# AlexandreDubray/consistent-viterbi

Measured on AMD Instinct MI355X. Metric: trellis cells/s (N*T*batch), N=256 T=512 batch=65536, higher is better.
Workload: dtype f64

## Files before the change

### consistent-viterbi_amd/csrc/cviterbi.cpp

```cpp
#include <hip/hip_runtime.h>

#include <algorithm>
#include <atomic>
#include <charconv>
#include <chrono>
#include <cmath>
#include <cstdarg>
#include <cstdio>
#include <cstdlib>
#include <cstring>
#include <memory>
#include <functional>
#include <limits>
#include <mutex>
#include <numeric>
#include <string>
#include <thread>
#include <type_traits>
#include <vector>

#include "../../include/cviterbi.h"
#include "batchplan.hpp"
#include "csp.hpp"
#include "hostscan.hpp"
// ... 3978 lines not shown
  return CV_OK;
}

CV_API int32_t cv_last_t64_stats(const cv_hmm* h, int64_t* out, int32_t n) {
  if (!h || n < 0 || (n > 0 && !out)) {
    set_err(CV_EINVAL, "bad argument");
    return -1;
  }
  int64_t v[8];
  t64_stats_sum(h, v);
  for (int32_t q = 0; q < n && q < 8; ++q) out[q] = v[q];
  return 8;
}

CV_API int32_t cv_last_fixed_first_stats(const cv_hmm* h, int64_t* out, int32_t n) {
  if (!h || n < 0 || (n > 0 && !out)) {
    set_err(CV_EINVAL, "bad argument");
    return -1;
  }
  for (int32_t q = 0; q < n && q < 4; ++q) out[q] = h->fx_last[q];
  return 4;
}

CV_API int32_t cv_last_first_pass_kind(const cv_hmm* h) {
  if (!h) {
    set_err(CV_EINVAL, "null handle");
    return -1;
  }
  return h->fx_last_kind;
}

CV_API cv_status cv_f32ru_trace(cv_hmm* h, int64_t nseq, int64_t T, const int32_t* obs, float* rows, float* mu,
                                float* r, float* e_last, int32_t* path) {
  if (!h || !obs || !rows || !mu || !r || !e_last || !path) return set_err(CV_EINVAL, "null argument");
  if (nseq < 2 || T < 1 || nseq * T > (1 << 22)) return set_err(CV_EINVAL, "bad batch shape");
  CV_LOCK(h);
  cv_status st = set_device(h);
  if (st != CV_OK) return st;
  for (int64_t e = 0; e < nseq * T; ++e)
    if (obs[e] < 0 || obs[e] >= h->V) return set_err(CV_EINVAL, "observation out of range");
  if ((st = ensure_ru_tables(h)) != CV_OK) return st;
  if (h->ru_state != 1) return set_err(CV_EINVAL, "the model is outside the round-up pass's range");
  const int np = cvk::trellis_padded_states(h->N);
  const size_t ne = (size_t)(nseq * T);
  std::vector<int64_t> off((size_t)nseq + 1);
  for (int64_t s = 0; s <= nseq; ++s) off[(size_t)s] = s * T;
  DevBuf d_off, d_obs, d_rows, d_mu, d_r, d_e, d_path, d_cert;
  if ((st = upload(d_off, off.data(), off.size() * 8)) != CV_OK) return st;
  if ((st = upload(d_obs, obs, ne * 4)) != CV_OK) return st;
  if ((st = d_rows.ensure(ne * np * 4)) != CV_OK) return st;
  if ((st = d_mu.ensure(ne * 4)) != CV_OK) return st;
  if ((st = d_r.ensure(ne * 4)) != CV_OK) return st;
  if ((st = d_e.ensure((size_t)nseq * 4)) != CV_OK) return st;
  if ((st = d_path.ensure(ne * 4)) != CV_OK) return st;
  if ((st = d_cert.ensure((size_t)nseq)) != CV_OK) return st;
  hipStream_t stream = h->stream;
  HIP_TRY(hipMemsetAsync(d_cert.p, 0, (size_t)nseq, stream));
  HIP_TRY(hipMemsetAsync(d_mu.p, 0, ne * 4, stream));
  HIP_TRY(hipMemsetAsync(d_r.p, 0, ne * 4, stream));
  HIP_TRY(hipMemsetAsync(d_rows.p, 0, ne * np * 4, stream));
  HIP_TRY(hipMemsetAsync(d_path.p, 0, ne * 4, stream));
  HIP_TRY(hipMemsetAsync(d_e.p, 0, (size_t)nseq * 4, stream));
  cvk::RuFwdArgs fa{};
  fa.a_img = h->ru_aimg.as<float>();
  fa.pi = h->ru_pi.as<float>();
  fa.et = h->ru_et.as<float>();
  fa.offsets = d_off.as<int64_t>();
  fa.obs = d_obs.as<int32_t>();
  fa.rows = d_rows.as<float>();
  fa.mu = d_mu.as<float>();
  fa.cert = d_cert.as<uint8_t>();
  fa.nobs = (int)h->V;
  hipError_t err = cvk::launch_ru_fwd2(np, fa, nseq / 2, stream);
  cvk::RuBtArgs ba{};
  ba.rows = fa.rows;
  ba.at = h->ru_at.as<float>();
  ba.offsets = fa.offsets;
  ba.seq_end = nseq - (nseq & 1);
  ba.path = d_path.as<int32_t>();
// ... 1631 lines not shown
```

### consistent-viterbi_amd/csrc/kernels/trellis.h

```cpp
#pragma once
#include <hip/hip_runtime.h>
#include <stdint.h>

namespace cvk {

enum { CVK_SEQ_OK = 0, CVK_SEQ_INFEASIBLE = 1, CVK_SEQ_EMPTY = 2, CVK_SEQ_BADOBS = 3 };
enum { CVK_ASSOC_VITERBI = 0, CVK_ASSOC_CP = 1, CVK_ASSOC_DP = 2, CVK_ASSOC_DECODE = 3 };

struct TrellisFwdArgs {
  const float* a_img;
  const float* pi;
  const float* et;
  const int64_t* offsets;
  const int32_t* obs;
  const int32_t* order;
  int64_t seq_begin;
  float* delta;
  int64_t delta_elem_base;
  uint8_t* status;
  int nobs;
  const int32_t* forced;
  const int64_t* ranges;
  int reverse;
  float* last_row;
// ... 96 lines not shown
  int nobs;
};
struct RuBtArgs {
  const float* rows;
  int64_t row_elem_base;
  const float* at;
  const int64_t* offsets;
  const int32_t* order;
  int64_t seq_begin, seq_end;
  int32_t* path;
  float* r;
  float* e_last;
  uint8_t* cert;
};
struct RuScoreArgs {
  const int32_t* path;
  const int32_t* obs;
  const int64_t* offsets;
  int64_t seq_begin, seq_end;
  int nstates;
  const double* pi64;
  const double* a64;
  const double* et64;
  const double* ca;
  const double* cb;
  const float* mu;
  const float* r;
  const float* e_last;
  double ks;
  uint8_t* cert;
  double* score;
  uint8_t* status;
};
hipError_t launch_ru_fwd2(int np, const RuFwdArgs& fa, int64_t npairs, hipStream_t stream);
hipError_t launch_ru_bt(int np, const RuBtArgs& ba, hipStream_t stream, int lds_reserve = 0);
hipError_t launch_ru_score(const RuScoreArgs& r, hipStream_t stream, int lds_reserve = 0);

template <typename REAL>
struct GenericFwdArgs {
  const int32_t* forced;
  const REAL* a;
  const REAL* pi;
  const REAL* et;
  const int64_t* offsets;
  const int32_t* obs;
  const int32_t* order;
  int64_t seq_begin;
  int nstates, nobs, assoc;
  uint16_t* psi;
  int64_t psi_elem_base;
  REAL* last_row;
  uint8_t* status;
  REAL* rows;
  const REAL* cp_init;
  REAL* cp_last;
  REAL* grows;
  int64_t wide_steps;
  int prio;
};

template <typename REAL>
struct GenericBtArgs {
  const uint16_t* psi;
  int64_t psi_elem_base;
  const REAL* last_row;
  const int64_t* offsets;
// ... 91 lines not shown
```

### consistent-viterbi_amd/csrc/kernels/trellis.hip

```cpp
#include <hip/hip_runtime.h>
#include <stdint.h>
#include <stdlib.h>

#include <algorithm>

#include "trellis.h"
#include "../tuning.h"

namespace cvk {

__device__ __forceinline__ float ninf_f() { return -__builtin_inff(); }

__device__ __forceinline__ float octet_max(float x) {
  asm volatile(
      "s_nop 1\n\t"
      "v_max_f32_dpp %0, %0, %0 quad_perm:[1,0,3,2] row_mask:0xf bank_mask:0xf\n\t"
      "s_nop 1\n\t"
      "v_max_f32_dpp %0, %0, %0 quad_perm:[2,3,0,1] row_mask:0xf bank_mask:0xf\n\t"
      "s_nop 1\n\t"
      "v_max_f32_dpp %0, %0, %0 row_half_mirror row_mask:0xf bank_mask:0xf"
      : "+v"(x));
  return x;
}

__device__ __forceinline__ float swap_max(float x, bool sixteen) {
  float a = x, b = x;
  if (sixteen)
    asm volatile("s_nop 1\n\tv_permlane16_swap_b32 %0, %1" : "+v"(a), "+v"(b));
  else
    asm volatile("s_nop 1\n\tv_permlane32_swap_b32 %0, %1" : "+v"(a), "+v"(b));
  return fmaxf(a, b);
}

__device__ __forceinline__ float wave_max(float x) {
  x = octet_max(x);
  asm volatile(
      "s_nop 1\n\t"
// ... 1015 lines not shown
}

hipError_t launch_fix_bt(int np, const FixBtArgs& ba, hipStream_t stream, int lds_reserve) {
  const int64_t n = ba.seq_end - ba.seq_begin;
  if (n <= 0) return hipSuccess;
  if (np != 256) return hipErrorInvalidValue;
  if (lds_reserve > 0)
    (void)hipFuncSetAttribute(reinterpret_cast<const void*>(&backtrack_fix_i32<256>),
                              hipFuncAttributeMaxDynamicSharedMemorySize, 160 * 1024);
  hipLaunchKernelGGL((backtrack_fix_i32<256>), dim3((unsigned)((n + 3) / 4)), dim3(256), (size_t)lds_reserve, stream,
                     ba);
  return hipGetLastError();
}

hipError_t launch_fix_score(const FixScoreArgs& r, hipStream_t stream, int lds_reserve) {
  const int64_t n = r.seq_end - r.seq_begin;
  if (n <= 0) return hipSuccess;
  if (lds_reserve > 0)
    (void)hipFuncSetAttribute(reinterpret_cast<const void*>(&fix_score_f64), hipFuncAttributeMaxDynamicSharedMemorySize,
                              160 * 1024);
  hipLaunchKernelGGL(fix_score_f64, dim3((unsigned)((n + 63) / 64)), dim3(64), (size_t)lds_reserve, stream, r);
  return hipGetLastError();
}

__device__ __forceinline__ void round_f32_up() {
  __builtin_amdgcn_s_setreg(1 | (1 << 11), 1);
  asm volatile("" ::: "memory");
}
__device__ __forceinline__ float dpp_max_half_mirror(float x) {
  asm volatile("s_nop 1\n\tv_max_f32_dpp %0, %0, %0 row_half_mirror row_mask:0xf bank_mask:0xf" : "+v"(x));
  return x;
}

template <int NP>
__global__ __launch_bounds__(NP * 4) void trellis_fwd2_f32ru(RuFwdArgs args) {
  using G = TrellisGeom<NP>;
  constexpr int R = G::R;
  constexpr int S = G::S;
  static_assert(R % 8 == 0, "pair kernel needs NP % 64 == 0");
  __shared__ __attribute__((aligned(16))) float lds[2][2][G::LDS_FLOATS];
  __shared__ float mu[2][3];
  round_f32_up();

  const int lane = threadIdx.x & 63;
  const int w = threadIdx.x >> 6;
  const int rg = lane & 7;
  const int cp = lane >> 3;
  const int j0 = 16 * w + 2 * cp;
  const bool hi = rg >= 4;
  const unsigned jw = (unsigned)(j0 + (hi ? 1 : 0));

  const int64_t slot = args.seq_begin + 2 * (int64_t)blockIdx.x;
  const int64_t seqX = args.order ? (int64_t)args.order[slot] : slot;
  const int64_t seqY = args.order ? (int64_t)args.order[slot + 1] : slot + 1;
  const int64_t eX = args.offsets[seqX], eY = args.offsets[seqY];
  const int T = (int)(args.offsets[seqX + 1] - eX);
  if (T <= 0) return;
  typedef const __attribute__((address_space(4))) int32_t* cobs_t;
  const cobs_t obsX = (cobs_t)(args.obs + eX);
  const cobs_t obsY = (cobs_t)(args.obs + eY);
  float* const dX = args.rows + (eX - args.row_elem_base) * NP;
  float* const dY = args.rows + (eY - args.row_elem_base) * NP;
  float* const muX = args.mu + eX;
  float* const muY = args.mu + eY;
  const unsigned V = (unsigned)args.nobs;

  if (threadIdx.x < 6) (&mu[0][0])[threadIdx.x] = ninf_f();
  __builtin_amdgcn_s_setprio(3);
// ... 26 lines not shown
  auto clampT = [&](int t) { return t < T ? t : T - 1; };
  typedef __attribute__((address_space(3))) float* lds_float_t;
  auto post_max = [&](float v, float* dst) {
    const float m = dpp_max_half_mirror(v);
    if (rg == 0) asm volatile("ds_max_f32 %0, %1" : : "v"((unsigned)(size_t)(lds_float_t)dst), "v"(m) : "memory");
  };
  lds_barrier();

  float eXr;
  {
    const float ex = et_row(obs_x(0)), ey = et_row(obs_y(0));
    const float p = args.pi[jw];
    eXr = et_row(obs_x(clampT(1)));
    const float dx = p + ex, dy = p + ey;
    lds[0][0][lds_w] = dx;
    lds[1][0][lds_w] = dy;
    dX[jw] = dx;
    dY[jw] = dy;
    post_max(dx, &mu[0][0]);
    post_max(dy, &mu[1][0]);
  }
  float eYr;
  unsigned oY = obs_y(clampT(1));
  unsigned oX = obs_x(clampT(2));
  lds_barrier();
  constexpr int KB = R / 8;
  auto ld8 = [&](const float* src, float4 (&dst)[2]) {
    dst[0] = *reinterpret_cast<const float4*>(src);
    dst[1] = *reinterpret_cast<const float4*>(src + 4);
  };
  float4 P[2], Q[2];
  ld8(&lds[0][0][rg * S], P);

  auto half = [&](const float* dsrc, const float* nsrc, float* ldst, float* drow, float* mus, float* mrow, int t,
                  const float& e_use, float& e_load, unsigned& o_load, bool first, int t_obs) {
    e_load = et_row(o_load);
    const float mu_use = fmaxf(mus[(t + 2) % 3], -__FLT_MAX__);
    if (threadIdx.x == 0) mus[(t + 1) % 3] = ninf_f();
    if (KB > 1) ld8(dsrc + 8, Q);
    float m0a = ninf_f(), m0b = ninf_f(), m1a = ninf_f(), m1b = ninf_f();
    auto rows4 = [&](const float4& dd, int k, bool init) {
      const float s00 = dd.x + a_reg[2 * k + 0], s01 = dd.x + a_reg[2 * k + 1];
      const float s10 = dd.y + a_reg[2 * k + 2], s11 = dd.y + a_reg[2 * k + 3];
      const float s20 = dd.z + a_reg[2 * k + 4], s21 = dd.z + a_reg[2 * k + 5];
      const float s30 = dd.w + a_reg[2 * k + 6], s31 = dd.w + a_reg[2 * k + 7];
      if (init) {
        m0a = fmaxf(s00, s10);
        m1a = fmaxf(s01, s11);
        m0b = fmaxf(s20, s30);
        m1b = fmaxf(s21, s31);
      } else {
        m0a = fmaxf(fmaxf(m0a, s00), s10);
        m1a = fmaxf(fmaxf(m1a, s01), s11);
        m0b = fmaxf(fmaxf(m0b, s20), s30);
        m1b = fmaxf(fmaxf(m1b, s21), s31);
      }
    };
#pragma unroll
    for (int k = 0; k < KB; ++k) {
      float4(&B)[2] = (k & 1) ? Q : P;
      rows4(B[0], 8 * k, k == 0);
      rows4(B[1], 8 * k + 4, false);
      __builtin_amdgcn_sched_barrier(0);
      if (k + 2 < KB)
        ld8(dsrc + 8 * (k + 2), B);
      else if (!(k & 1) && (k + 2 == KB || k + 1 == KB) && !first)
        ld8(nsrc, P);
      __builtin_amdgcn_sched_barrier(0);
    }
    const float m0 = fmaxf(m0a, m0b);
    const float m1 = fmaxf(m1a, m1b);
    float m = dpp_max_mirror(hi ? m1 : m0, hi ? m0 : m1);
    m = dpp_max_xor1(m);
    m = dpp_max_xor2(m);
    const float dn = (m + e_use) - mu_use;
    __builtin_amdgcn_sched_barrier(0);
    o_load = first ? obs_y(t_obs) : obs_x(t_obs);
    ldst[lds_w] = dn;
    (drow + (size_t)t * NP)[jw] = dn;
    mrow[t] = mu_use;
    post_max(dn, &mus[t % 3]);
    if (first) {
      lds_barrier();
      ld8(nsrc, P);
    }
  };
  auto step = [&](int t) {
    const int cur = (t - 1) & 1, nxt = t & 1;
    half(&lds[0][cur][rg * S], &lds[1][cur][rg * S], &lds[0][nxt][0], dX, mu[0], muX, t, eXr, eYr, oY, true,
         clampT(t + 1));
    half(&lds[1][cur][rg * S], &lds[0][nxt][rg * S], &lds[1][nxt][0], dY, mu[1], muY, t, eYr, eXr, oX, false,
         clampT(t + 2));
  };
  for (int t = 1; t < T; ++t) step(t);
  if (bad && lane == 0 && w == 0) {
    if (bad & 1u) args.cert[seqX] = CVK_SEQ_BADOBS;
    if (bad & 2u) args.cert[seqY] = CVK_SEQ_BADOBS;
  }
}

template <int NP>
__global__ __launch_bounds__(256) void backtrack_f32ru(RuBtArgs args) {
  constexpr int VL = NP / 64;
  constexpr int PF = 8;
  static_assert(VL == 4, "float4 rows");
  round_f32_up();
  const int lane = threadIdx.x & 63;
  const int64_t slot = args.seq_begin + (int64_t)blockIdx.x * 4 + (threadIdx.x >> 6);
  if (slot >= args.seq_end) return;
  const int64_t seq = args.order ? (int64_t)args.order[slot] : slot;
  const int64_t e0 = args.offsets[seq];
  const int T = (int)(args.offsets[seq + 1] - e0);
  if (T <= 0 || args.cert[seq] != 0) return;
  int32_t* __restrict__ path = args.path + e0;
  float* __restrict__ rout = args.r + e0;
  const float* __restrict__ drow = args.rows + (e0 - args.row_elem_base) * NP + VL * lane;
  const float* __restrict__ at = args.at + VL * lane;
  auto load_row = [&](int r, float (&dst)[VL]) {
    if (r >= 0) {
      ld_vl<VL>(drow + (size_t)r * NP, dst);
    } else {
      dst[0] = dst[1] = dst[2] = dst[3] = ninf_f();
    }
  };
  auto top2 = [&](const float (&s)[VL], float& M2) -> int {
    const float M = wave_max(fmaxf(fmaxf(s[0], s[1]), fmaxf(s[2], s[3])));
    const int win = first_argmax_vl<VL>(s, M, lane) & (NP - 1);
// ... 50 lines not shown
  const int32_t* __restrict__ obs = r.obs + e0;
  const float* __restrict__ mu = r.mu + e0;
  const float* __restrict__ rr = r.r + e0;
  const int N = r.nstates;
  auto absfin = [](double x) { return __builtin_isinf(x) ? 0.0 : __builtin_fabs(x); };
  auto sigma = [&](int n, double s) { return r.ks * (((double)n + 2.0) * ((double)n + 2.0)) + 0x1p-49 * s; };
  int pp = path[0];
  double L = r.pi64[pp] + r.et64[(size_t)obs[0] * N + pp];
  double C = r.cb[obs[0]];
  bool ok = true;
  for (int t = 1; t < T; ++t) {
    const int p = path[t];
    const int o = obs[t];
    const double rt = (double)rr[t], cap = r.ca[p];
    const double lhs = L + r.a64[(size_t)pp * N + p];
    const double rhs = (rt + cap) + C;
    ok = ok && (lhs - rhs > sigma(t, absfin(rt) + __builtin_fabs(cap) + __builtin_fabs(C) + __builtin_fabs(lhs)));
    L = lhs + r.et64[(size_t)o * N + p];
    const double ct = r.cb[o], mt = (double)mu[t];
    const double s = __builtin_fabs(C) + __builtin_fabs(ct) + __builtin_fabs(mt);
    C = ((C + ct) + mt) + 0x1p-50 * s;
    pp = p;
  }
  const double E = (double)r.e_last[seq];
  ok = ok && (L - (E + C) > sigma(T, absfin(E) + __builtin_fabs(C) + __builtin_fabs(L)));
  if (ok) {
    r.score[seq] = L;
    r.status[seq] = CVK_SEQ_OK;
  } else {
    r.cert[seq] = 2;
  }
}

hipError_t launch_ru_fwd2(int np, const RuFwdArgs& fa, int64_t npairs, hipStream_t stream) {
  if (npairs <= 0) return hipSuccess;
  if (np != 256) return hipErrorInvalidValue;
  hipLaunchKernelGGL((trellis_fwd2_f32ru<256>), dim3((unsigned)npairs), dim3(1024), 0, stream, fa);
  return hipGetLastError();
}

hipError_t launch_ru_bt(int np, const RuBtArgs& ba, hipStream_t stream, int lds_reserve) {
  const int64_t n = ba.seq_end - ba.seq_begin;
  if (n <= 0) return hipSuccess;
  if (np != 256) return hipErrorInvalidValue;
  if (lds_reserve > 0)
    (void)hipFuncSetAttribute(reinterpret_cast<const void*>(&backtrack_f32ru<256>),
                              hipFuncAttributeMaxDynamicSharedMemorySize, 160 * 1024);
  hipLaunchKernelGGL((backtrack_f32ru<256>), dim3((unsigned)((n + 3) / 4)), dim3(256), (size_t)lds_reserve, stream, ba);
  return hipGetLastError();
}

hipError_t launch_ru_score(const RuScoreArgs& r, hipStream_t stream, int lds_reserve) {
  const int64_t n = r.seq_end - r.seq_begin;
  if (n <= 0) return hipSuccess;
  if (lds_reserve > 0)
    (void)hipFuncSetAttribute(reinterpret_cast<const void*>(&ru_score_f64), hipFuncAttributeMaxDynamicSharedMemorySize,
                              160 * 1024);
  hipLaunchKernelGGL(ru_score_f64, dim3((unsigned)((n + 63) / 64)), dim3(64), (size_t)lds_reserve, stream, r);
  return hipGetLastError();
}

template <int NPW, bool FRC>
__global__ __launch_bounds__(256) void trellis_wave_f32(TrellisFwdArgs args, BacktrackArgs bargs) {
  constexpr int C = NPW / 16;
  constexpr int R = NPW / 4;
  constexpr int LS = R + 4;
  static_assert(NPW % 16 == 0 && NPW >= 16 && NPW <= 64, "NPW in {16, 32, 48, 64}");
  __shared__ __attribute__((aligned(16))) float lds_all[4][2][4 * LS];
  __shared__ __attribute__((aligned(16))) float at_lds[NPW * NPW];
  for (int k = threadIdx.x; k < NPW * NPW; k += 256) at_lds[k] = bargs.at[k];
// ... 1410 lines not shown
```

### consistent-viterbi_amd/csrc/tuning.cpp

```cpp
#include "tuning.h"

#include <cctype>
#include <cstdlib>
#include <cstring>
#include <string>

namespace cvk {
namespace {

struct Key {
  const char* name;
  int Tuning::*field;
};

#define CVK_KEY(f) {#f, &Tuning::f}
const Key kKeys[] = {
    CVK_KEY(trace), CVK_KEY(host_threads), CVK_KEY(t64_nonpos), CVK_KEY(generic_rows),
    CVK_KEY(max_chunks), CVK_KEY(emis_overlap), CVK_KEY(host_sums), CVK_KEY(no_trace), CVK_KEY(no_resume),
    CVK_KEY(no_side), CVK_KEY(chain_par), CVK_KEY(chain_old), CVK_KEY(chain_par_force),
    CVK_KEY(chain_spec), CVK_KEY(chain_spec_kernel), CVK_KEY(chain_copy_overlap), CVK_KEY(chain_cert_fused),
    CVK_KEY(chain_parts), CVK_KEY(chain_tail), CVK_KEY(chain_tail_div), CVK_KEY(chain_spec_prio), CVK_KEY(chain_pin_obs), CVK_KEY(chain_pin_path), CVK_KEY(t64_s),
    CVK_KEY(t64_512), CVK_KEY(t64_1024), CVK_KEY(t64_wg), CVK_KEY(t64_wg_force),
    CVK_KEY(t64_rs), CVK_KEY(t64_w2), CVK_KEY(t64_wave), CVK_KEY(t64_bal),
    CVK_KEY(t64_cp_s), CVK_KEY(t64_cp_w), CVK_KEY(t64_cp_pf), CVK_KEY(t64_bt_pf),
    CVK_KEY(t64_lo_every), CVK_KEY(t64_fixed_first), CVK_KEY(t64_fixed_chunks), CVK_KEY(t64_few),
    CVK_KEY(t64_f32ru_first),
    CVK_KEY(generic_s), CVK_KEY(generic_split), CVK_KEY(generic_split_k), CVK_KEY(generic_wide),
    CVK_KEY(generic_wide_min), CVK_KEY(generic_prio), CVK_KEY(wide_s), CVK_KEY(ext_wide_min),
    CVK_KEY(chain_wide), CVK_KEY(chain_wide_min), CVK_KEY(f32_onebar), CVK_KEY(bw_global),
    CVK_KEY(bw_perseq), CVK_KEY(bw_gemm_path), CVK_KEY(bw_chunk_elems), CVK_KEY(bw_max_waves),
    CVK_KEY(xi_part_rows),
};
#undef CVK_KEY

const Key* find(const char* key) {
  if (!key) return nullptr;
  for (const Key& k : kKeys)
    if (std::strcmp(k.name, key) == 0) return &k;
  return nullptr;
}

const Tuning kDefaults{};
thread_local const Tuning* t_cur = nullptr;
thread_local Tuning t_copy;
thread_local int t_depth = 0;

}

const Tuning& tuning() { return t_cur ? *t_cur : kDefaults; }

void tuning_enter(const Tuning& t) {
  if (t_depth++ == 0) {
    t_copy = t;
    t_cur = &t_copy;
  }
}

void tuning_leave() {
  if (t_depth > 0 && --t_depth == 0) t_cur = nullptr;
// ... 46 lines not shown
```

### consistent-viterbi_amd/csrc/tuning.h

```cpp
#pragma once

#include <cstdint>

namespace cvk {

struct Tuning {
  int trace = 0;
  int host_threads = 0;
  int t64_nonpos = 1;
  int generic_rows = 1;
  int max_chunks = 8;
  int emis_overlap = 0;
  int host_sums = 0;
  int no_trace = 0;
  int no_resume = 0;
  int no_side = 0;
  int chain_par = 1;
  int chain_old = 0;
  int chain_par_force = 0;
  int chain_spec = 1;
  int chain_spec_kernel = 0;
  int chain_copy_overlap = 1;
  int chain_cert_fused = 1;
  int chain_parts = 1;
  int chain_tail = 2;
  int chain_tail_div = 2;
  int chain_spec_prio = 3;
  int chain_pin_obs = 0;
  int chain_pin_path = 0;
  int t64_s = 0;
  int t64_512 = -1;
  int t64_1024 = -1;
  int t64_wg = 1;
  int t64_wg_force = 0;
  int t64_rs = 1;
  int t64_w2 = 1;
  int t64_few = -1;
  int t64_wave = 1;
  int t64_bal = 8;
  int t64_cp_s = 0;
  int t64_cp_pf = 0;
  int t64_cp_w = 0;
  int t64_bt_pf = 0;
  int t64_lo_every = 8;
  int t64_fixed_first = 16777216;
  int t64_f32ru_first = 16777216;
  int t64_fixed_chunks = 8;
  int generic_s = 0;
  int generic_split = 0;
  int generic_split_k = 0;
  int generic_wide = 1;
  int generic_wide_min = 0;
  int generic_prio = 0;
  int wide_s = 0;
  int ext_wide_min = 0;
  int chain_wide = 1;
  int chain_wide_min = 0;
  int f32_onebar = 1;
  int bw_global = 0;
  int bw_perseq = 0;
  int bw_gemm_path = 0;
  int bw_chunk_elems = 0;
  int bw_max_waves = 0;
  int xi_part_rows = 0;
};

const Tuning& tuning();
void tuning_enter(const Tuning& t);
void tuning_leave();
struct TuningOverride {
  TuningOverride(int Tuning::*field, int value);
  ~TuningOverride();
  TuningOverride(const TuningOverride&) = delete;
  TuningOverride& operator=(const TuningOverride&) = delete;

 private:
  int Tuning::*field_;
  int saved_;
  bool on_;
// ... 15 lines not shown
```

### consistent-viterbi_amd/cviterbi/__init__.py

```python
from ._lib import CVError, EXPORTS, LIB_PATH
from .hmm import HMM, tuning_keys
from .decode import (constrained_pairs, constrained_partials, constrained_select, decode, decode_batch, decode_batch_device, decode_constrained_device, decode_constrained_exchange,
                     decode_constrained, decode_forced_components, decode_superseq_cp, device_memory, f32ru_trace, last_first_pass_kind, last_suffix_traced, last_fixed_first_stats, last_superseq_stats, last_t64_stats, last_timing, timing_begin,
                     timing_end)
from .counts import (expected_counts, expected_counts_device, expected_counts_emissions,
                     expected_counts_emissions_device, reestimate)
from .emissions import decode_emissions, decode_emissions_device
from .grad import loglik_grad_emissions, loglik_grad_emissions_device
from . import autograd
from .emissions import posterior_emissions, posterior_emissions_device, score_emissions
from .fit import fit_mle, fit_train, last_fit_stats
from .kbest import kbest_batch, kbest_batch_device
from .posterior import posterior_batch, posterior_batch_device, score_batch
from .sample import sample_batch, sample_batch_device, uniform
from .solver import (Constraints, GpuSolver, Solver, SuperSequence, load_sequences, load_tags,
                     write_output)
```

### consistent-viterbi_amd/cviterbi/_lib.py

```python
from __future__ import annotations

import ctypes
import os

_HERE = os.path.dirname(os.path.abspath(__file__))
LIB_PATH = os.environ.get("CV_LIB_PATH") or os.path.join(_HERE, "libcviterbi.so")

(CV_OK, CV_EINVAL, CV_EDEVICE, CV_ENOMEM, CV_EINFEASIBLE, CV_EIO, CV_EPARSE, CV_EUNSUPPORTED, CV_EINTERNAL,
 CV_ELIMIT) = range(10)
STATUS_NAMES = {0: "CV_OK", 1: "CV_EINVAL", 2: "CV_EDEVICE", 3: "CV_ENOMEM", 4: "CV_EINFEASIBLE", 5: "CV_EIO",
                6: "CV_EPARSE", 7: "CV_EUNSUPPORTED", 8: "CV_EINTERNAL", 9: "CV_ELIMIT"}
SEQ_OK, SEQ_INFEASIBLE, SEQ_EMPTY, SEQ_BADOBS = 0, 1, 2, 3
DTYPE_F32, DTYPE_F64 = 0, 1
ASSOC_VITERBI, ASSOC_CP, ASSOC_DP, ASSOC_DECODE = 0, 1, 2, 3
KERNEL_AUTO, KERNEL_TRELLIS, KERNEL_GENERIC, KERNEL_TRELLIS_F64 = 0, 1, 2, 3
FLAG_NO_PAIR = 0x4
FLAG_NO_WAVE = 0x8
FLAG_NO_T64 = 0x10
FLAG_SERIAL = 0x2


EXPORTS = [
    "cv_last_error", "cv_version", "cv_abi_version", "cv_device_count", "cv_device_memory", "cv_opts_init",
    "cv_hmm_create", "cv_hmm_from_json", "cv_hmm_write_json", "cv_hmm_destroy", "cv_hmm_nstates", "cv_hmm_nobs",
    "cv_hmm_ndims", "cv_hmm_bdims", "cv_obs_flatten", "cv_hmm_init_prob", "cv_hmm_init_probs",
    "cv_hmm_transition_prob", "cv_hmm_transitions_to", "cv_hmm_emit_prob", "cv_hmm_emit_probs",
    "cv_decode_batch", "cv_decode_batch_device", "cv_last_timing", "cv_timing_begin", "cv_timing_end",
    "cv_decode_constrained", "cv_decode_constrained_device", "cv_last_suffix_traced", "cv_decode_constrained_exchange",
    "cv_constrained_pairs", "cv_constrained_partials", "cv_constrained_select", "cv_decode_forced_components", "cv_viterbi_decode",
    "cv_decode_superseq_cp", "cv_last_superseq_stats",
    "cv_solver_create", "cv_solver_solve", "cv_solver_get_solution", "cv_solver_get_objective",
    "cv_solver_get_name", "cv_solver_get_explored_nodes", "cv_solver_destroy",
    "cv_hmm_fit_mle", "cv_hmm_fit_train", "cv_solver_write_cfn",
    "cv_hmm_set_tuning", "cv_hmm_get_tuning", "cv_tuning_key", "cv_hmm_release_workspaces",
    "cv_posterior_batch", "cv_posterior_batch_device",
    "cv_kbest_batch", "cv_kbest_batch_device",
    "cv_decode_emissions", "cv_decode_emissions_device",
    "cv_posterior_emissions", "cv_posterior_emissions_device",
    "cv_expected_counts", "cv_expected_counts_device",
    "cv_expected_counts_emissions", "cv_expected_counts_emissions_device",
    "cv_loglik_grad_emissions", "cv_loglik_grad_emissions_device",
    "cv_sample_batch", "cv_sample_batch_device",
    "cv_last_t64_stats", "cv_last_fixed_first_stats", "cv_hmm_fit_last_stats",
    "cv_last_first_pass_kind", "cv_f32ru_trace",
]


class CVError(RuntimeError):
    def __init__(self, status, message):
        super().__init__(f"{STATUS_NAMES.get(status, status)}: {message}")
        self.status = status


class HmmDesc(ctypes.Structure):
    _fields_ = [("nstates", ctypes.c_int32), ("ndims", ctypes.c_int32), ("bdims", ctypes.c_void_p),
                ("pi", ctypes.c_void_p), ("a", ctypes.c_void_p), ("b", ctypes.c_void_p), ("device", ctypes.c_int32)]


class Opts(ctypes.Structure):
    _fields_ = [("dtype", ctypes.c_int32), ("assoc", ctypes.c_int32), ("kernel", ctypes.c_int32),
                ("rescore_f64", ctypes.c_int32), ("stream", ctypes.c_void_p), ("workspace_bytes", ctypes.c_uint64),
                ("flags", ctypes.c_uint32), ("forced", ctypes.c_void_p)]


class Timing(ctypes.Structure):
    _fields_ = [("fwd_ms", ctypes.c_double), ("bt_ms", ctypes.c_double), ("total_ms", ctypes.c_double),
                ("launches", ctypes.c_int64), ("kernel", ctypes.c_int32), ("padded_states", ctypes.c_int32),
                ("mfma_tiles", ctypes.c_int32)]


class SuperSeqDesc(ctypes.Structure):
    _fields_ = [("nseq", ctypes.c_int64), ("offsets", ctypes.c_void_p), ("obs", ctypes.c_void_p),
                ("seq_id", ctypes.c_void_p), ("component", ctypes.c_void_p), ("active", ctypes.c_void_p)]


_lib = None

# ... 41 lines not shown
        "cv_posterior_batch_device": ([P, I64, P, P, P, P, P, P, P, P], S),
        "cv_sample_batch": ([P, I64, P, P, I32, ctypes.c_uint64, I64, P, P, P, P, P], S),
        "cv_sample_batch_device": ([P, I64, P, P, P, I32, ctypes.c_uint64, I64, P, P, P, P, P], S),
        "cv_kbest_batch": ([P, I64, P, P, I32, P, P, P, P, P], S),
        "cv_kbest_batch_device": ([P, I64, P, P, P, I32, P, P, P, P, P], S),
        "cv_decode_emissions": ([P, I64, P, P, I64, P, P, P, P], S),
        "cv_decode_emissions_device": ([P, I64, P, P, P, I64, P, P, P, P], S),
        "cv_posterior_emissions": ([P, I64, P, P, I64, P, P, P, P, P], S),
        "cv_posterior_emissions_device": ([P, I64, P, P, P, I64, P, P, P, P, P], S),
        "cv_expected_counts": ([P, I64, P, P, P, P, P, P, P, P], S),
        "cv_expected_counts_device": ([P, I64, P, P, P, P, P, P, P, P, P], S),
        "cv_expected_counts_emissions": ([P, I64, P, P, I64, P, P, P, P, P, P], S),
        "cv_expected_counts_emissions_device": ([P, I64, P, P, P, I64, P, P, P, P, P, P], S),
        "cv_loglik_grad_emissions": ([P, I64, P, P, I64, P, P, P, P, P, P, I64, P], S),
        "cv_loglik_grad_emissions_device": ([P, I64, P, P, P, I64, P, P, P, P, P, P, I64, P], S),
        "cv_last_timing": ([P, P], S),
        "cv_timing_begin": ([P], S),
        "cv_timing_end": ([P, P], S),
        "cv_last_suffix_traced": ([P, P], S),
        "cv_decode_constrained": ([P, I64, P, P, P, I32, P, P, P, P, P, P], S),
        "cv_decode_constrained_device": ([P, I64, P, P, P, P, I32, P, P, P, P, P, P], S),
        "cv_decode_constrained_exchange": ([P, I64, P, P, P, I32, I64, P, P, P, P, P, P, P, P, P, P], S),
        "cv_constrained_pairs": ([I64, P, P, I32, P, I64, P], S),
        "cv_constrained_partials": ([P, I64, P, P, P, I32, I64, P, P, P], S),
        "cv_constrained_select": ([I32, I32, I64, P, P, P, P], S),
        "cv_decode_forced_components": ([P, I64, P, P, P, I32, P, P, P, P, P, P], S),
        "cv_viterbi_decode": ([P, I64, P, P], S),
        "cv_decode_superseq_cp": ([P, I64, P, P, P, P], S),
        "cv_last_superseq_stats": ([P, P], S),
        "cv_last_t64_stats": ([P, P, I32], I32),
        "cv_last_fixed_first_stats": ([P, P, I32], I32),
        "cv_last_first_pass_kind": ([P], I32),
        "cv_f32ru_trace": ([P, I64, I64, P, P, P, P, P, P], S),
        "cv_device_memory": ([P, P], S),
        "cv_solver_create": ([ctypes.c_char_p, P, P, P], S),
        "cv_solver_solve": ([P], S),
        "cv_solver_get_solution": ([P, P, P], S),
        "cv_solver_get_objective": ([P, P], S),
        "cv_solver_get_name": ([P], ctypes.c_char_p),
        "cv_solver_get_explored_nodes": ([P, P], S),
        "cv_solver_destroy": ([P], None),
        "cv_solver_write_cfn": ([P, ctypes.c_char_p, P], S),
        "cv_hmm_fit_mle": ([I32, I64, I64, P, P, P, I32, P, P, P], S),
        "cv_hmm_fit_train": ([I32, I64, I64, P, P, P, I32, D, I32, P, P, P, P], S),
        "cv_hmm_fit_last_stats": ([P, I32], I32),
    }
    for name, (args, res) in sig.items():
        f = getattr(L, name)
        f.argtypes = args
        f.restype = res
    _lib = L
    return L


def check(status):
    if status != CV_OK:
        raise CVError(status, lib().cv_last_error().decode())


def opts(dtype=DTYPE_F32, assoc=ASSOC_VITERBI, kernel=KERNEL_AUTO, rescore_f64=True, stream=None,
         workspace_bytes=0, flags=0):
    o = Opts()
    lib().cv_opts_init(ctypes.byref(o))
    o.dtype, o.assoc, o.kernel, o.rescore_f64 = dtype, assoc, kernel, int(bool(rescore_f64))
    o.stream = stream
    o.workspace_bytes = workspace_bytes
# ... 3 lines not shown
```

### consistent-viterbi_amd/cviterbi/decode.py

```python
from __future__ import annotations

import ctypes

import numpy as np

from . import _lib as L
from .hmm import HMM

_DT = {"f32": L.DTYPE_F32, "f64": L.DTYPE_F64, np.float32: L.DTYPE_F32, np.float64: L.DTYPE_F64}
_ASSOC = {"viterbi": L.ASSOC_VITERBI, "cp": L.ASSOC_CP, "dp": L.ASSOC_DP, "decode": L.ASSOC_DECODE}
_KERNEL = {"auto": L.KERNEL_AUTO, "trellis": L.KERNEL_TRELLIS, "generic": L.KERNEL_GENERIC,
           "trellis_f64": L.KERNEL_TRELLIS_F64}


def _p(x):
    return x.ctypes.data_as(ctypes.c_void_p)


def make_opts(dtype="f64", assoc="viterbi", kernel="auto", rescore_f64=True, stream=None, workspace_bytes=0,
              variant=None, serial=False):
    flags = L.FLAG_SERIAL if serial else 0
    if variant == "valu1":
        flags |= L.FLAG_NO_PAIR | L.FLAG_NO_WAVE
    elif variant == "nowave":
# ... 207 lines not shown
FIXED_FIRST_STATS = ("engaged", "certified", "fallback", "pinned")


def last_fixed_first_stats(hmm: HMM) -> dict:
    out = (ctypes.c_int64 * len(FIXED_FIRST_STATS))()
    n = L.lib().cv_last_fixed_first_stats(hmm.handle, out, len(FIXED_FIRST_STATS))
    if n < 0:
        L.check(L.CV_EINVAL)
    return {k: int(out[i]) for i, k in enumerate(FIXED_FIRST_STATS[:n])}


FIRST_PASS_KINDS = ("none", "fixed", "f32ru")


def last_first_pass_kind(hmm: HMM) -> str:
    k = L.lib().cv_last_first_pass_kind(hmm.handle)
    if k < 0:
        L.check(L.CV_EINVAL)
    return FIRST_PASS_KINDS[k]


def f32ru_trace(hmm: HMM, obs) -> dict:
    obs = np.ascontiguousarray(obs, np.int32)
    S, T = obs.shape
    N = hmm.nstates()
    rows = np.empty((S, T, N), np.float32)
    mu, r = np.empty((S, T), np.float32), np.empty((S, T), np.float32)
    E, path = np.empty(S, np.float32), np.empty((S, T), np.int32)
    ptr = lambda x: x.ctypes.data_as(ctypes.c_void_p)
    L.check(L.lib().cv_f32ru_trace(hmm.handle, S, T, ptr(obs), ptr(rows), ptr(mu), ptr(r), ptr(E), ptr(path)))
    return dict(rows=rows.transpose(1, 0, 2), mu=mu, r=r, E=E, path=path)


def device_memory() -> dict:
    cur, peak = ctypes.c_int64(), ctypes.c_int64()
    L.check(L.lib().cv_device_memory(ctypes.byref(cur), ctypes.byref(peak)))
    return dict(current=cur.value, peak=peak.value)


def _timing_dict(t):
    return dict(fwd_ms=t.fwd_ms, bt_ms=t.bt_ms, total_ms=t.total_ms, launches=t.launches,
                kernel={1: "trellis", 2: "generic", 3: "trellis_f64"}.get(t.kernel, "none"), padded_states=t.padded_states,
                seqs_per_wave=t.mfma_tiles)


def last_suffix_traced(hmm: HMM) -> int:
    n = ctypes.c_int64()
    L.check(L.lib().cv_last_suffix_traced(hmm.handle, ctypes.byref(n)))
    return n.value


def last_timing(hmm: HMM) -> dict:
    t = L.Timing()
    L.check(L.lib().cv_last_timing(hmm.handle, ctypes.byref(t)))
    return _timing_dict(t)


def timing_begin(hmm: HMM):
    L.check(L.lib().cv_timing_begin(hmm.handle))


def timing_end(hmm: HMM) -> dict:
    t = L.Timing()
    L.check(L.lib().cv_timing_end(hmm.handle, ctypes.byref(t)))
    return _timing_dict(t)

# ... 7 lines not shown
```

### include/cviterbi.h

```cpp
#ifndef CVITERBI_H
#define CVITERBI_H

#include <stddef.h>
#include <stdint.h>

#ifdef __cplusplus
extern "C" {
#endif

#define CV_API __attribute__((visibility("default")))
#define CV_ABI_VERSION 1

typedef enum cv_status {
  CV_OK = 0,
  CV_EINVAL = 1,
  CV_EDEVICE = 2,
  CV_ENOMEM = 3,
  CV_EINFEASIBLE = 4,
  CV_EIO = 5,
  CV_EPARSE = 6,
  CV_EUNSUPPORTED = 7,
  CV_EINTERNAL = 8,
  CV_ELIMIT = 9
} cv_status;
// ... 64 lines not shown
CV_API cv_status cv_hmm_create(const cv_hmm_desc* desc, cv_hmm** out);
CV_API cv_status cv_hmm_from_json(const char* path, int32_t device, cv_hmm** out);
CV_API cv_status cv_hmm_write_json(const cv_hmm* h, const char* path);
CV_API void cv_hmm_destroy(cv_hmm* h);
CV_API cv_status cv_hmm_release_workspaces(cv_hmm* h);
CV_API cv_status cv_hmm_set_tuning(cv_hmm* h, const char* key, int64_t value);
CV_API cv_status cv_hmm_get_tuning(const cv_hmm* h, const char* key, int64_t* value);
CV_API const char* cv_tuning_key(int32_t i);

CV_API int32_t cv_hmm_nstates(const cv_hmm* h);
CV_API int64_t cv_hmm_nobs(const cv_hmm* h);
CV_API int32_t cv_hmm_ndims(const cv_hmm* h);
CV_API cv_status cv_hmm_bdims(const cv_hmm* h, int64_t* bdims_out );
CV_API cv_status cv_obs_flatten(const cv_hmm* h, const int64_t* value , int64_t* flat_out);
CV_API double cv_hmm_init_prob(const cv_hmm* h, int32_t state, int64_t obs);
CV_API cv_status cv_hmm_init_probs(const cv_hmm* h, int64_t obs, double* out);
CV_API double cv_hmm_transition_prob(const cv_hmm* h, int32_t from, int32_t to, int64_t obs);
CV_API cv_status cv_hmm_transitions_to(const cv_hmm* h, int32_t to, double* out);
CV_API double cv_hmm_emit_prob(const cv_hmm* h, int32_t state, int64_t obs);
CV_API cv_status cv_hmm_emit_probs(const cv_hmm* h, int64_t obs, double* out);

CV_API cv_status cv_decode_batch(cv_hmm* h, int64_t nseq, const int64_t* offsets, const int32_t* obs,
                                 const cv_opts* opts, int32_t* path_out, double* score_out,
                                 uint8_t* status_out);
CV_API cv_status cv_decode_batch_device(cv_hmm* h, int64_t nseq, const int64_t* offsets_host,
                                        const int64_t* offsets_dev, const int32_t* obs_dev,
                                        const cv_opts* opts, int32_t* path_dev, double* score_dev,
                                        uint8_t* status_dev);
CV_API int32_t cv_last_t64_stats(const cv_hmm* h, int64_t* out, int32_t n);
CV_API int32_t cv_last_fixed_first_stats(const cv_hmm* h, int64_t* out, int32_t n);
CV_API int32_t cv_last_first_pass_kind(const cv_hmm* h);
CV_API cv_status cv_f32ru_trace(cv_hmm* h, int64_t nseq, int64_t T, const int32_t* obs, float* rows, float* mu,
                                float* r, float* e_last, int32_t* path);
CV_API cv_status cv_last_timing(cv_hmm* h, cv_timing* out);
CV_API cv_status cv_timing_begin(cv_hmm* h);
CV_API cv_status cv_timing_end(cv_hmm* h, cv_timing* out);
CV_API cv_status cv_decode_constrained(cv_hmm* h, int64_t nseq, const int64_t* offsets, const int32_t* obs,
                                       const int32_t* component, int32_t ncomp, const cv_opts* opts,
                                       int32_t* path_out, double* score_out, uint8_t* status_out,
                                       int32_t* comp_state_out, double* objective_out);
CV_API cv_status cv_decode_constrained_device(cv_hmm* h, int64_t nseq, const int64_t* offsets_host,
                                              const int64_t* offsets_dev, const int32_t* obs_dev,
                                              const int32_t* component, int32_t ncomp, const cv_opts* opts,
                                              int32_t* path_dev, double* score_dev, uint8_t* status_dev,
                                              int32_t* comp_state_out, double* objective_out);
CV_API cv_status cv_last_suffix_traced(const cv_hmm* h, int64_t* out);
#define CV_PARTIAL_WORDS(nstates, ncomp, npairs) \
  ((int64_t)(ncomp) * (5 * (int64_t)(nstates) + 1) + (int64_t)(npairs) * (5 * (int64_t)(nstates) * (nstates) + 1))
CV_API cv_status cv_constrained_pairs(int64_t nseq, const int64_t* offsets, const int32_t* component, int32_t ncomp,
                                      int32_t* pairs_out, int64_t cap_pairs, int64_t* npairs_out);
CV_API cv_status cv_constrained_partials(cv_hmm* h, int64_t nseq, const int64_t* offsets, const int32_t* obs,
                                         const int32_t* component, int32_t ncomp, int64_t npairs,
                                         const int32_t* pairs, const cv_opts* opts, int64_t* partials_out);
CV_API cv_status cv_constrained_select(int32_t nstates, int32_t ncomp, int64_t npairs, const int32_t* pairs,
                                       const int64_t* partials, int32_t* comp_state_out, uint64_t* explored_out);
CV_API cv_status cv_decode_forced_components(cv_hmm* h, int64_t nseq, const int64_t* offsets, const int32_t* obs,
                                             const int32_t* component, int32_t ncomp, const int32_t* comp_state,
                                             const cv_opts* opts, int32_t* path_out, double* score_out,
                                             uint8_t* status_out, double* objective_out);
typedef int32_t (*cv_exchange_fn)(int64_t* words, int64_t nwords, void* ctx);
CV_API cv_status cv_decode_constrained_exchange(cv_hmm* h, int64_t nseq, const int64_t* offsets, const int32_t* obs,
                                                const int32_t* component, int32_t ncomp, int64_t npairs,
                                                const int32_t* pairs, cv_exchange_fn exchange, void* ctx,
                                                const cv_opts* opts, int32_t* path_out, double* score_out,
                                                uint8_t* status_out, int32_t* comp_state_out,
                                                uint64_t* explored_out, double* objective_out);
// ... 97 lines not shown
```

Baseline: 81.33 billion.

## Measure f32 round-up row max every K steps and predict drift in between

The f32 round-up forward kernel now takes a template parameter K and posts and reads the per-row maximum through LDS only every K steps. In the steps between, it uses a normaliser extrapolated from the last measured max divided by K, made wave-uniform with readfirstlane. It also advances the delta row pointer incrementally instead of recomputing the index, and adds a ragged-offsets trace entry point. The aim is to cut the LDS max reduction and its synchronisation on most time steps, at the cost of normalisers that are only approximate between measurements, which the later score or certification stages have to absorb.

```diff
diff --git a/consistent-viterbi_amd/csrc/cviterbi.cpp b/consistent-viterbi_amd/csrc/cviterbi.cpp
--- a/consistent-viterbi_amd/csrc/cviterbi.cpp
+++ b/consistent-viterbi_amd/csrc/cviterbi.cpp
@@ -4034,19 +4034,31 @@
 
 CV_API cv_status cv_f32ru_trace(cv_hmm* h, int64_t nseq, int64_t T, const int32_t* obs, float* rows, float* mu,
                                 float* r, float* e_last, int32_t* path) {
-  if (!h || !obs || !rows || !mu || !r || !e_last || !path) return set_err(CV_EINVAL, "null argument");
   if (nseq < 2 || T < 1 || nseq * T > (1 << 22)) return set_err(CV_EINVAL, "bad batch shape");
+  std::vector<int64_t> off((size_t)nseq + 1);
+  for (int64_t s = 0; s <= nseq; ++s) off[(size_t)s] = s * T;
+  return cv_f32ru_trace_ragged(h, nseq, off.data(), obs, rows, mu, r, e_last, path);
+}
+
+CV_API cv_status cv_f32ru_trace_ragged(cv_hmm* h, int64_t nseq, const int64_t* offsets, const int32_t* obs,
+                                       float* rows, float* mu, float* r, float* e_last, int32_t* path) {
+  if (!h || !offsets || !obs || !rows || !mu || !r || !e_last || !path) return set_err(CV_EINVAL, "null argument");
+  if (nseq < 2 || nseq > (1 << 22) || offsets[0] != 0) return set_err(CV_EINVAL, "bad batch shape");
+  for (int64_t s = 0; s < nseq; ++s) {
+    const int64_t len = offsets[s + 1] - offsets[s];
+    if (len < 1 || offsets[s + 1] > (1 << 22)) return set_err(CV_EINVAL, "bad batch shape");
+    if ((s & 1) && len != offsets[s] - offsets[s - 1]) return set_err(CV_EINVAL, "a pair of two lengths");
+  }
   CV_LOCK(h);
   cv_status st = set_device(h);
   if (st != CV_OK) return st;
-  for (int64_t e = 0; e < nseq * T; ++e)
+  const size_t ne = (size_t)offsets[nseq];
+  for (size_t e = 0; e < ne; ++e)
     if (obs[e] < 0 || obs[e] >= h->V) return set_err(CV_EINVAL, "observation out of range");
   if ((st = ensure_ru_tables(h)) != CV_OK) return st;
   if (h->ru_state != 1) return set_err(CV_EINVAL, "the model is outside the round-up pass's range");
   const int np = cvk::trellis_padded_states(h->N);
-  const size_t ne = (size_t)(nseq * T);
-  std::vector<int64_t> off((size_t)nseq + 1);
-  for (int64_t s = 0; s <= nseq; ++s) off[(size_t)s] = s * T;
+  const std::vector<int64_t> off(offsets, offsets + nseq + 1);
   DevBuf d_off, d_obs, d_rows, d_mu, d_r, d_e, d_path, d_cert;
   if ((st = upload(d_off, off.data(), off.size() * 8)) != CV_OK) return st;
   if ((st = upload(d_obs, obs, ne * 4)) != CV_OK) return st;
diff --git a/consistent-viterbi_amd/csrc/kernels/trellis.h b/consistent-viterbi_amd/csrc/kernels/trellis.h
--- a/consistent-viterbi_amd/csrc/kernels/trellis.h
+++ b/consistent-viterbi_amd/csrc/kernels/trellis.h
@@ -152,6 +152,7 @@
   double* score;
   uint8_t* status;
 };
+int ru_mu_every();
 hipError_t launch_ru_fwd2(int np, const RuFwdArgs& fa, int64_t npairs, hipStream_t stream);
 hipError_t launch_ru_bt(int np, const RuBtArgs& ba, hipStream_t stream, int lds_reserve = 0);
 hipError_t launch_ru_score(const RuScoreArgs& r, hipStream_t stream, int lds_reserve = 0);
diff --git a/consistent-viterbi_amd/csrc/kernels/trellis.hip b/consistent-viterbi_amd/csrc/kernels/trellis.hip
--- a/consistent-viterbi_amd/csrc/kernels/trellis.hip
+++ b/consistent-viterbi_amd/csrc/kernels/trellis.hip
@@ -3,6 +3,7 @@
 #include <stdlib.h>
 
 #include <algorithm>
+#include <type_traits>
 
 #include "trellis.h"
 #include "../tuning.h"
@@ -1084,8 +1085,9 @@
   return x;
 }
 
-template <int NP>
+template <int NP, int K>
 __global__ __launch_bounds__(NP * 4) void trellis_fwd2_f32ru(RuFwdArgs args) {
+  static_assert(K >= 1 && (K & (K - 1)) == 0, "the predictor divides by K exactly");
   using G = TrellisGeom<NP>;
   constexpr int R = G::R;
   constexpr int S = G::S;
@@ -1178,12 +1180,22 @@
   float4 P[2], Q[2];
   ld8(&lds[0][0][rg * S], P);
 
-  auto half = [&](const float* dsrc, const float* nsrc, float* ldst, float* drow, float* mus, float* mrow, int t,
-                  const float& e_use, float& e_load, unsigned& o_load, bool first, int t_obs) {
+  auto half = [&](const float* dsrc, const float* nsrc, float* ldst, float*& drow, float* mus, float* mrow, int t,
+                  const float& e_use, float& e_load, unsigned& o_load, float& dhat, int sr, auto first_c,
+                  bool meas, bool post, int t_obs) {
+    constexpr bool first = decltype(first_c)::value;
     e_load = et_row(o_load);
-    const float mu_use = fmaxf(mus[(t + 2) % 3], -__FLT_MAX__);
-    if (threadIdx.x == 0) mus[(t + 1) % 3] = ninf_f();
     if (KB > 1) ld8(dsrc + 8, Q);
+    float mu_use = dhat;
+    if (meas) {
+      const float m_raw = fmaxf(mus[sr], -0x1p126f);
+      if (threadIdx.x == 0) mus[sr == 0 ? 2 : sr - 1] = ninf_f();
+      const float d = dhat + (t > 1 && fabsf(m_raw) >= 0x1p-64f ? m_raw * (1.0f / K) : 0.0f);
+      dhat = __builtin_bit_cast(float, __builtin_amdgcn_readfirstlane(
+                                           __builtin_bit_cast(int, fabsf(d) < 64.0f ? d : 0.0f)));
+      mu_use = m_raw + dhat;
+    }
+    float emu = 0.0f;
     float m0a = ninf_f(), m0b = ninf_f(), m1a = ninf_f(), m1b = ninf_f();
     auto rows4 = [&](const float4& dd, int k, bool init) {
       const float s00 = dd.x + a_reg[2 * k + 0], s01 = dd.x + a_reg[2 * k + 1];
@@ -1213,32 +1225,43 @@
       else if (!(k & 1) && (k + 2 == KB || k + 1 == KB) && !first)
         ld8(nsrc, P);
       __builtin_amdgcn_sched_barrier(0);
+      if (k == (KB > 1 ? 1 : 0)) {
+        emu = e_use - mu_use;
+        mrow[t] = mu_use;
+      }
     }
     const float m0 = fmaxf(m0a, m0b);
     const float m1 = fmaxf(m1a, m1b);
     float m = dpp_max_mirror(hi ? m1 : m0, hi ? m0 : m1);
     m = dpp_max_xor1(m);
     m = dpp_max_xor2(m);
-    const float dn = (m + e_use) - mu_use;
+    const float dn = m + emu;
     __builtin_amdgcn_sched_barrier(0);
     o_load = first ? obs_y(t_obs) : obs_x(t_obs);
     ldst[lds_w] = dn;
-    (drow + (size_t)t * NP)[jw] = dn;
-    mrow[t] = mu_use;
-    post_max(dn, &mus[t % 3]);
+    drow += NP;
+    *drow = dn;
+    if (post) post_max(dn, &mus[sr == 2 ? 0 : sr + 1]);
     if (first) {
       lds_barrier();
       ld8(nsrc, P);
     }
   };
-  auto step = [&](int t) {
+  float dhX = 0.0f, dhY = 0.0f;
+  float* pX = dX + jw;
+  float* pY = dY + jw;
+  auto step = [&](int t, int sr, bool meas, bool post) {
     const int cur = (t - 1) & 1, nxt = t & 1;
-    half(&lds[0][cur][rg * S], &lds[1][cur][rg * S], &lds[0][nxt][0], dX, mu[0], muX, t, eXr, eYr, oY, true,
-         clampT(t + 1));
-    half(&lds[1][cur][rg * S], &lds[0][nxt][rg * S], &lds[1][nxt][0], dY, mu[1], muY, t, eYr, eXr, oX, false,
-         clampT(t + 2));
-  };
-  for (int t = 1; t < T; ++t) step(t);
+    half(&lds[0][cur][rg * S], &lds[1][cur][rg * S], &lds[0][nxt][0], pX, mu[0], muX, t, eXr, eYr, oY, dhX, sr,
+         std::true_type{}, meas, post, clampT(t + 1));
+    half(&lds[1][cur][rg * S], &lds[0][nxt][rg * S], &lds[1][nxt][0], pY, mu[1], muY, t, eYr, eXr, oX, dhY, sr,
+         std::false_type{}, meas, post, clampT(t + 2));
+  };
+  for (int t = 1, sr = 0; t < T; ++t) {
+    const bool post = (t & (K - 1)) == 0;
+    step(t, sr, ((t - 1) & (K - 1)) == 0, post);
+    if (post) sr = __builtin_amdgcn_readfirstlane(sr == 2 ? 0 : sr + 1);
+  }
   if (bad && lane == 0 && w == 0) {
     if (bad & 1u) args.cert[seqX] = CVK_SEQ_BADOBS;
     if (bad & 2u) args.cert[seqY] = CVK_SEQ_BADOBS;
@@ -1355,10 +1378,21 @@
   }
 }
 
+int ru_mu_every() {
+  const int v = tuning().t64_f32ru_mu_every;
+  if (v <= 0) return Tuning{}.t64_f32ru_mu_every;
+  return v <= 2 ? 1 : v <= 6 ? 4 : 8;
+}
+
 hipError_t launch_ru_fwd2(int np, const RuFwdArgs& fa, int64_t npairs, hipStream_t stream) {
   if (npairs <= 0) return hipSuccess;
   if (np != 256) return hipErrorInvalidValue;
-  hipLaunchKernelGGL((trellis_fwd2_f32ru<256>), dim3((unsigned)npairs), dim3(1024), 0, stream, fa);
+  const dim3 grid((unsigned)npairs), block(1024);
+  switch (ru_mu_every()) {
+    case 1: hipLaunchKernelGGL((trellis_fwd2_f32ru<256, 1>), grid, block, 0, stream, fa); break;
+    case 4: hipLaunchKernelGGL((trellis_fwd2_f32ru<256, 4>), grid, block, 0, stream, fa); break;
+    default: hipLaunchKernelGGL((trellis_fwd2_f32ru<256, 8>), grid, block, 0, stream, fa); break;
+  }
   return hipGetLastError();
 }
 
diff --git a/consistent-viterbi_amd/csrc/tuning.cpp b/consistent-viterbi_amd/csrc/tuning.cpp
--- a/consistent-viterbi_amd/csrc/tuning.cpp
+++ b/consistent-viterbi_amd/csrc/tuning.cpp
@@ -24,7 +24,7 @@
     CVK_KEY(t64_rs), CVK_KEY(t64_w2), CVK_KEY(t64_wave), CVK_KEY(t64_bal),
     CVK_KEY(t64_cp_s), CVK_KEY(t64_cp_w), CVK_KEY(t64_cp_pf), CVK_KEY(t64_bt_pf),
     CVK_KEY(t64_lo_every), CVK_KEY(t64_fixed_first), CVK_KEY(t64_fixed_chunks), CVK_KEY(t64_few),
-    CVK_KEY(t64_f32ru_first),
+    CVK_KEY(t64_f32ru_first), CVK_KEY(t64_f32ru_mu_every),
     CVK_KEY(generic_s), CVK_KEY(generic_split), CVK_KEY(generic_split_k), CVK_KEY(generic_wide),
     CVK_KEY(generic_wide_min), CVK_KEY(generic_prio), CVK_KEY(wide_s), CVK_KEY(ext_wide_min),
     CVK_KEY(chain_wide), CVK_KEY(chain_wide_min), CVK_KEY(f32_onebar), CVK_KEY(bw_global),
diff --git a/consistent-viterbi_amd/csrc/tuning.h b/consistent-viterbi_amd/csrc/tuning.h
--- a/consistent-viterbi_amd/csrc/tuning.h
+++ b/consistent-viterbi_amd/csrc/tuning.h
@@ -45,6 +45,7 @@
   int t64_lo_every = 8;
   int t64_fixed_first = 16777216;
   int t64_f32ru_first = 16777216;
+  int t64_f32ru_mu_every = 4;
   int t64_fixed_chunks = 8;
   int generic_s = 0;
   int generic_split = 0;
diff --git a/consistent-viterbi_amd/cviterbi/__init__.py b/consistent-viterbi_amd/cviterbi/__init__.py
--- a/consistent-viterbi_amd/cviterbi/__init__.py
+++ b/consistent-viterbi_amd/cviterbi/__init__.py
@@ -1,7 +1,7 @@
 from ._lib import CVError, EXPORTS, LIB_PATH
 from .hmm import HMM, tuning_keys
 from .decode import (constrained_pairs, constrained_partials, constrained_select, decode, decode_batch, decode_batch_device, decode_constrained_device, decode_constrained_exchange,
-                     decode_constrained, decode_forced_components, decode_superseq_cp, device_memory, f32ru_trace, last_first_pass_kind, last_suffix_traced, last_fixed_first_stats, last_superseq_stats, last_t64_stats, last_timing, timing_begin,
+                     decode_constrained, decode_forced_components, decode_superseq_cp, device_memory, f32ru_trace, f32ru_trace_ragged, last_first_pass_kind, last_suffix_traced, last_fixed_first_stats, last_superseq_stats, last_t64_stats, last_timing, timing_begin,
                      timing_end)
 from .counts import (expected_counts, expected_counts_device, expected_counts_emissions,
                      expected_counts_emissions_device, reestimate)
diff --git a/consistent-viterbi_amd/cviterbi/_lib.py b/consistent-viterbi_amd/cviterbi/_lib.py
--- a/consistent-viterbi_amd/cviterbi/_lib.py
+++ b/consistent-viterbi_amd/cviterbi/_lib.py
@@ -42,7 +42,7 @@
     "cv_loglik_grad_emissions", "cv_loglik_grad_emissions_device",
     "cv_sample_batch", "cv_sample_batch_device",
     "cv_last_t64_stats", "cv_last_fixed_first_stats", "cv_hmm_fit_last_stats",
-    "cv_last_first_pass_kind", "cv_f32ru_trace",
+    "cv_last_first_pass_kind", "cv_f32ru_trace", "cv_f32ru_trace_ragged",
 ]
 
 
@@ -150,6 +150,7 @@
         "cv_last_fixed_first_stats": ([P, P, I32], I32),
         "cv_last_first_pass_kind": ([P], I32),
         "cv_f32ru_trace": ([P, I64, I64, P, P, P, P, P, P], S),
+        "cv_f32ru_trace_ragged": ([P, I64, P, P, P, P, P, P, P], S),
         "cv_device_memory": ([P, P], S),
         "cv_solver_create": ([ctypes.c_char_p, P, P, P], S),
         "cv_solver_solve": ([P], S),
diff --git a/consistent-viterbi_amd/cviterbi/decode.py b/consistent-viterbi_amd/cviterbi/decode.py
--- a/consistent-viterbi_amd/cviterbi/decode.py
+++ b/consistent-viterbi_amd/cviterbi/decode.py
@@ -263,6 +263,20 @@
     return dict(rows=rows.transpose(1, 0, 2), mu=mu, r=r, E=E, path=path)
 
 
+def f32ru_trace_ragged(hmm: HMM, offsets, obs) -> dict:
+    offsets = np.ascontiguousarray(offsets, np.int64)
+    obs = np.ascontiguousarray(obs, np.int32)
+    S, ne, N = len(offsets) - 1, int(offsets[-1]), hmm.nstates()
+    assert obs.shape == (ne,)
+    rows = np.empty((ne, N), np.float32)
+    mu, r = np.empty(ne, np.float32), np.empty(ne, np.float32)
+    E, path = np.empty(S, np.float32), np.empty(ne, np.int32)
+    ptr = lambda x: x.ctypes.data_as(ctypes.c_void_p)
+    L.check(L.lib().cv_f32ru_trace_ragged(hmm.handle, S, ptr(offsets), ptr(obs), ptr(rows), ptr(mu), ptr(r), ptr(E),
+                                          ptr(path)))
+    return dict(rows=rows, mu=mu, r=r, E=E, path=path)
+
+
 def device_memory() -> dict:
     cur, peak = ctypes.c_int64(), ctypes.c_int64()
     L.check(L.lib().cv_device_memory(ctypes.byref(cur), ctypes.byref(peak)))
diff --git a/include/cviterbi.h b/include/cviterbi.h
--- a/include/cviterbi.h
+++ b/include/cviterbi.h
@@ -120,6 +120,8 @@
 CV_API int32_t cv_last_first_pass_kind(const cv_hmm* h);
 CV_API cv_status cv_f32ru_trace(cv_hmm* h, int64_t nseq, int64_t T, const int32_t* obs, float* rows, float* mu,
                                 float* r, float* e_last, int32_t* path);
+CV_API cv_status cv_f32ru_trace_ragged(cv_hmm* h, int64_t nseq, const int64_t* offsets, const int32_t* obs,
+                                       float* rows, float* mu, float* r, float* e_last, int32_t* path);
 CV_API cv_status cv_last_timing(cv_hmm* h, cv_timing* out);
 CV_API cv_status cv_timing_begin(cv_hmm* h);
 CV_API cv_status cv_timing_end(cv_hmm* h, cv_timing* out);
```

Result: faster. 88.08 billion, median of 6 (+8.3%).
